# tunabrain/tungsten

Measured on AMD Instinct MI355X. Metric: Msamples/s (W*H*spp/s), path_tracer render loop, higher is better.
Workload: dtype f32; 1 GPU; materialtest.json (3 meshes 80768 tris + quad, smooth_coat/rough_conductor/lambert, envmap MIS) 1280x720 @ 256 spp; width=1280, height=720, spp=256, sampler=uniform (counter-based PCG), adaptive_sampling=False, max_bounces=64, parallelism=tile-shard x1

## Files before the change

tungsten_amd/csrc/hip/pt_wavefront.h:

```cpp
#ifndef TGAMD_PT_WAVEFRONT_H_
#define TGAMD_PT_WAVEFRONT_H_
#include "pt_kernels.h"

#include <hip/hip_runtime.h>

#include <cstdio>
#include <cstdlib>
#include <cstring>
#include <mutex>
#include <string>
#include <type_traits>
#include <vector>


#ifdef PT_PROFILE
#define PROF_DECL unsigned long long profT = wall_clock64(), profAcc[16] = {0, 0, 0, 0, 0, 0, 0, 0, 0, 0, 0, 0, 0, 0, 0, 0}, profLn[16] = {0, 0, 0, 0, 0, 0, 0, 0, 0, 0, 0, 0, 0, 0, 0, 0}
#define PROF(n) do { unsigned long long t_ = wall_clock64(); profAcc[n] += t_ - profT; profLn[n] += (t_ - profT)*(unsigned long long)__popcll(__ballot(true)); profT = t_; if ((n) == 0) profAcc[10]++; } while (0)
#define PROF_FLUSH(stats) do { if (laneId() == 0) for (int k_ = 0; k_ < 16; ++k_) if (k_ != 11) { if (k_ != 10) atomicAdd(&(stats).prof[k_], profAcc[k_]); atomicAdd(&(stats).profCls[cls][k_], profAcc[k_]); atomicAdd(&(stats).profLanes[cls][k_], profLn[k_]); } } while (0)
#else
#define PROF_DECL
#define PROF(n)
#define PROF_FLUSH(stats)
#endif

// ... 315 lines not shown
        }
        if (busyMask == 0ull)
            break;
        bool pop = false;
        if (busy && cur >= 0) {
            const float4 *nd = &at32(s.nodes, (uint32_t)cur*4u);
            float4 n0 = ld4(nd, 0u), n1 = ld4(nd, 1u), n2 = ld4(nd, 2u), n3 = ld4(nd, 3u);
            if (COUNT) nodes++;
            float e0, e1;
            bool h0 = boxTest(mk3(n0.x, n0.y, n0.z), mk3(n0.w, n1.x, n1.y), ray, invD, tmax, e0);
            bool h1 = boxTest(mk3(n1.z, n1.w, n2.x), mk3(n2.y, n2.z, n2.w), ray, invD, tmax, e1);
            int c0 = __float_as_int(n3.x), c1 = __float_as_int(n3.y);
            if (h0 && h1) {
                if (e1 < e0) { stack[sp*stride] = c0; cur = c1; }
                else { stack[sp*stride] = c1; cur = c0; }
                sp++;
            } else if (h0) { cur = c0; }
            else if (h1) { cur = c1; }
            else pop = true;
        }
        {
            unsigned long long atLeaf = __ballot(busy && cur < 0 && !pop);
            unsigned long long atNode = __ballot(busy && (cur >= 0 || pop));
            if (atLeaf != 0ull && ((uint32_t)__popcll(atLeaf) >= st.leaf_batch_bvh2 || atNode == 0ull)) {
                if (busy && cur < 0 && !pop) {
                    uint32_t firstRec = TGHIP_LEAF_FIRST(cur), count = TGHIP_LEAF_COUNT(cur);
                    for (uint32_t r = firstRec; r < firstRec + count; ++r) {
                        if (COUNT) prims++;
                        uint32_t meta;
                        (void)testRecord<false, SOLIDS ? KINDS_ALL : KINDS_MESH>(s, r, ray, tmax, hit, meta);
                    }
                    pop = true;
                }
            }
        }
        if (busy && pop) {
            if (sp == 0) {
                slotF4(st, A_HIT, slot) = hit;
                int ri = __float_as_int(hit.w);
                int cls = ri < 0 ? CLS_MISS : (int)at32(s.rec_class, (uint32_t)ri);
                queuePush(true, local, L, shadeQueue(cls));
                busy = false;
            } else {
                sp--;
                cur = stack[sp*stride];
            }
        }
    }
    waveAddStat(&L.closest_rays, rays);
    if (COUNT) { waveAddStat(&L.nodes, nodes); waveAddStat(&L.prims, prims); }
    queuesEnd(L, st, Q_EXT, Q_SHADE_MASK, Q_EXTP);
    if (threadIdx.x == 0) {
        ctl.closest_rays += L.closest_rays;
        if (COUNT) { st.stats[blockIdx.x].nodes_visited += L.nodes; st.stats[blockIdx.x].prims_tested += L.prims; }
    }
}

template<bool COUNT, bool SOLIDS = true>
__global__ __launch_bounds__(512) void k_trace_closest_inst(DeviceScene s, PathState st)
{
    extern __shared__ int ldsDyn[];
    __shared__ BlockLdsSmall L;
    __shared__ uint32_t fetchNext;
    unsigned short *order = reinterpret_cast<unsigned short *>(ldsDyn);
    int *stack = ldsDyn + (st.slots_per_block >> 1) + threadIdx.x;
    const int stride = (int)blockDim.x;
    BlockCtl &ctl = st.ctl[blockIdx.x];
    if (threadIdx.x == 0) fetchNext = 0;
    queuesBegin(L, st, ctl, Q_EXTP, 0u, order, Q_EXT);
    const uint32_t n = L.n;
    const uint32_t first = blockIdx.x*st.slots_per_block;
    uint32_t nodes = 0, prims = 0, rays = 0;
    constexpr uint32_t KINDS = SOLIDS ? KINDS_ALL : KINDS_MESH;

    bool busy = false;
    uint32_t slot = 0, local = 0;
    RayD world; world.o = splat3(0.0f); world.d = splat3(1.0f); world.tmin = 0.0f; world.tmax = 0.0f;
    RayD ray = world;
    f3 invD = splat3(1.0f), winvD = splat3(1.0f);
    float tmax = 0.0f;
    float4 hit = make_float4(0.0f, 0.0f, 0.0f, __int_as_float(-1));
    int hitInst = -1;
    int cur = 0, sp = 0, level = 0;
    float refTMin = 0.0f, refTMax = 0.0f, refFarT = 0.0f;
    int refSp = 0;
    uint32_t leafNext = 0, leafEnd = 0;
    int instSp = 0, curInst = -1;
    float ltmax = 0.0f;
    float4 lhit = hit;
    bool exhausted = false;
    uint32_t sec[24] = {0, 0, 0, 0, 0, 0, 0, 0, 0, 0, 0, 0, 0, 0, 0, 0, 0, 0, 0, 0, 0, 0, 0, 0};
#define INST_SECTION(k, pred) do { if (COUNT) { const unsigned long long m_ = __ballot(pred); if (m_) { sec[2*(k)]++; sec[2*(k) + 1] += (uint32_t)__popcll(m_); } } } while (0)
    for (;;) {
        unsigned long long busyMask = __ballot(busy);
        if (!exhausted && __popcll(busyMask) <= 48) {
            INST_SECTION(11, !busy);
            unsigned long long want = ~busyMask;
            uint32_t lane = laneId();
            uint32_t base = 0;
            if (lane == 0)
                base = atomicAdd(&fetchNext, (uint32_t)__popcll(want));
            base = __shfl(base, 0);
            if (!busy) {
                uint32_t i = base + __popcll(want & ((1ull << lane) - 1ull));
                if (i < n) {
                    local = order[i];
                    slot = first + local;
                    float4 ro = slotF4(st, A_RAY_O, slot), rd = slotF4(st, A_RAY_D, slot);
                    world.o = xyz(ro); world.d = xyz(rd); world.tmin = ro.w; world.tmax = rd.w;
                    ray = world;
                    winvD = mk3(1.0f/world.d.x, 1.0f/world.d.y, 1.0f/world.d.z);
                    invD = winvD;
                    tmax = world.tmax;
                    hit = make_float4(tmax, 0.0f, 0.0f, __int_as_float(-1));
                    hitInst = -1;
                    cur = 0; sp = 0; level = 0;
                    busy = true;
                    rays++;
                }
            }
            if (base + (uint32_t)__popcll(want) >= n)
                exhausted = true;
            busyMask = __ballot(busy);
        }
        if (busyMask == 0ull)
            break;
        bool pop = false;
        INST_SECTION(0, busy);
        INST_SECTION(1, busy && cur >= 0);
        INST_SECTION(2, busy && cur >= 0 && level == 1);
        if (busy && cur >= 0) {
            const float4 *nd = &at32(s.nodes, (uint32_t)cur*4u);
            const float4 n0 = ld4(nd, 0u), n1 = ld4(nd, 1u), n2 = ld4(nd, 2u), n3 = ld4(nd, 3u);
            if (COUNT) nodes++;
            const f3 lo0 = mk3(n0.x, n0.y, n0.z), hi0 = mk3(n0.w, n1.x, n1.y), lo1 = mk3(n1.z, n1.w, n2.x), hi1 = mk3(n2.y, n2.z, n2.w);
            const int c0 = __float_as_int(n3.x), c1 = __float_as_int(n3.y);
            float e0, e1;
            bool h0, h1, firstIs1;
            if (level == 1) {
                h0 = refChildTest(lo0, hi0, world.o, world.d, winvD, world.tmin, refFarT, e0);
                h1 = refChildTest(lo1, hi1, world.o, world.d, winvD, world.tmin, refFarT, e1);
                firstIs1 = !(e0 < e1);
            } else {
                const float far = level == 2 ? ltmax : tmax;
                h0 = boxTest(lo0, hi0, ray, invD, far, e0);
                h1 = boxTest(lo1, hi1, ray, invD, far, e1);
                firstIs1 = e1 < e0;
            }
            float entry = 0.0f;
            if (h0 && h1) {
                stack[sp*stride] = firstIs1 ? c0 : c1;
                sp++;
                cur = firstIs1 ? c1 : c0;
                entry = firstIs1 ? e1 : e0;
            } else if (h0) { cur = c0; entry = e0; }
            else if (h1) { cur = c1; entry = e1; }
            else pop = true;
            if (level == 1 && !pop) refTMin = entry;
        }
        {
            unsigned long long atLeaf = __ballot(busy && cur < 0 && !pop);
            unsigned long long atNode = __ballot(busy && (cur >= 0 || pop));
            if (atLeaf != 0ull && ((uint32_t)__popcll(atLeaf) >= st.leaf_batch_bvh2 || atNode == 0ull)) {
                INST_SECTION(3, busy && cur < 0 && !pop);
                INST_SECTION(4, busy && cur < 0 && !pop && level == 1);
                INST_SECTION(6, busy && cur < 0 && !pop && level != 1);
                if (busy && cur < 0 && !pop) {
                    if (level == 1) {
                        if (leafNext == leafEnd) { leafNext = TGHIP_LEAF_FIRST(cur); leafEnd = leafNext + TGHIP_LEAF_COUNT(cur); }
                        const uint32_t ri = s.inst_prims[leafNext];
                        leafNext++;
                        if (COUNT) prims++;
                        if (instanceReachable(s, ri, world, winvD, refTMin)) {
                            int root;
                            instanceLocalRay(s, ri, world, refTMin, PT_INF, ray, root);
                            invD = mk3(1.0f/ray.d.x, 1.0f/ray.d.y, 1.0f/ray.d.z);
                            ltmax = PT_INF;
                            lhit = make_float4(PT_INF, 0.0f, 0.0f, __int_as_float(-1));
                            curInst = (int)ri;
                            instSp = sp;
                            stack[sp*stride] = cur;
                            sp++;
                            cur = root;
                            level = 2;
                        } else if (leafNext == leafEnd) {
                            refTMax = refMin(refTMax, tmax);
                            refFarT = refTMax;
                            leafNext = leafEnd = 0;
                            pop = true;
                        }
                    } else {
                        const uint32_t firstRec = TGHIP_LEAF_FIRST(cur), count = TGHIP_LEAF_COUNT(cur);
                        bool entered = false;
                        if (level == 0) {
                            const float4 r0 = ld4(s.recs, firstRec*3u);
                            INST_SECTION(5, TGHIP_REC_KIND(__float_as_uint(r0.w)) == TGHIP_REC_INSTANCE_SET);
                            if (TGHIP_REC_KIND(__float_as_uint(r0.w)) == TGHIP_REC_INSTANCE_SET) {
                                if (COUNT) prims++;
                                const float4 r1 = ld4(s.recs, firstRec*3u + 1u), r2 = ld4(s.recs, firstRec*3u + 2u);
                                float tMin = world.tmin, tMax = tmax;
                                if (refBboxIntersection(xyz(r0), xyz(r1), world, tMin, tMax)) {
                                    refTMin = tMin; refTMax = tMax; refFarT = tmax;
                                    refSp = sp;
                                    leafNext = leafEnd = 0;
                                    cur = __float_as_int(r2.x);
                                    level = 1;
                                } else {
                                    pop = true;
                                }
                                entered = true;
                            }
                        }
                        if (!entered) {
                            for (uint32_t r = firstRec; r < firstRec + count; ++r) {
                                if (COUNT) prims++;
                                uint32_t meta;
                                if (level == 2) (void)testRecord<false, KINDS>(s, r, ray, ltmax, lhit, meta);
                                else if (testRecord<false, KINDS>(s, r, ray, tmax, hit, meta)) hitInst = -1;
                            }
                            pop = true;
                        }
                    }
                }
            }
        }
        INST_SECTION(7, busy && pop);
        INST_SECTION(8, busy && pop && level == 2 && sp == instSp + 1);
        if (busy && pop) {
            if (level == 2 && sp == instSp + 1) {
                if (__float_as_int(lhit.w) >= 0) { hit = lhit; hitInst = curInst; tmax = lhit.x; }
                ray = world; invD = winvD;
                level = 1;
                sp--;
                cur = stack[sp*stride];
                if (leafNext == leafEnd) {
                    refTMax = refMin(refTMax, tmax);
                    refFarT = refTMax;
                    leafNext = leafEnd = 0;
                } else {
                    pop = false;
                }
            }
            INST_SECTION(9, pop && level == 1);
            if (pop && level == 1) {
                for (;;) {
                    if (sp == refSp) { level = 0; break; }
                    sp--;
                    cur = stack[sp*stride];
                    if (cur >= 0) { pop = false; break; }
                    refTMin = refLeafEntry(s, TGHIP_LEAF_FIRST(cur), world.o, world.d, winvD, world.tmin);
                    if (!(refTMax < refTMin)) { pop = false; break; }
                }
            }
            INST_SECTION(10, pop && level != 1 && sp == 0);
            if (pop && level != 1) {
                if (sp == 0) {
                    slotF4(st, A_HIT, slot) = hit;
                    slotW(st, A_EMI, slot, 3u) = __int_as_float(hitInst);
                    int ri = __float_as_int(hit.w);
                    int cls = ri < 0 ? CLS_MISS : (int)at32(s.rec_class, (uint32_t)ri);
                    queuePush(true, local, L, shadeQueue(cls));
                    busy = false;
                } else {
                    sp--;
                    cur = stack[sp*stride];
                }
            }
        }
    }
    if (COUNT && laneId() == 0) {
        unsigned long long *wk = st.stats[blockIdx.x].walk[0];
        atomicAdd(&wk[4], 1ull);
        for (int k = 0; k < 24; ++k) atomicAdd(&wk[24 + k], (unsigned long long)sec[k]);
    }
#undef INST_SECTION
    waveAddStat(&L.closest_rays, rays);
    if (COUNT) { waveAddStat(&L.nodes, nodes); waveAddStat(&L.prims, prims); }
    queuesEnd(L, st, Q_EXT, Q_SHADE_MASK, Q_EXTP);
    if (threadIdx.x == 0) {
        ctl.closest_rays += L.closest_rays;
        if (COUNT) { st.stats[blockIdx.x].nodes_visited += L.nodes; st.stats[blockIdx.x].prims_tested += L.prims; }
    }
}

#ifndef PT_CLOSEST_WAVES
#define PT_CLOSEST_WAVES 5
#endif
#ifndef WIDE_CLOSEST_BOUNDS
#define WIDE_CLOSEST_BOUNDS __launch_bounds__(512, PT_CLOSEST_WAVES)
#endif
#ifndef WIDE_SHADOW_BOUNDS
#define WIDE_SHADOW_BOUNDS __launch_bounds__(512, 4)
#endif
#define PT_TURN_JOIN() asm volatile("" ::: "memory")
#define PT_WALK_FETCH(s, r0, r1, r2, nd, hasRec, recIdx, hasNode, nodeIdx) do { \
        const uint32_t recAt_ = (hasRec) ? (recIdx)*3u : 0u; \
        const uint32_t nodeAt_ = (hasNode) ? wideNodeOff(s, nodeIdx) : 0u; \
        r0 = at32((s).recs, recAt_); r1 = at32((s).recs, recAt_ + 1u); r2 = at32((s).recs, recAt_ + 2u); \
        wideNodeFetch(nd, reinterpret_cast<const char *>((s).wide), nodeAt_); \
    } while (0)
#ifndef PT_REFILL_AT
#define PT_REFILL_AT 40
#endif
template<bool COUNT, bool SOLIDS, bool INST, bool DECOUPLED, int NTS = PT_NT_STATE>
PT_DEV void traceClosestWideBody(const DeviceScene &s, const PathState &st, BlockLds &L, uint32_t &fetchNext, int *ldsDyn)
{
    unsigned short *order = reinterpret_cast<unsigned short *>(ldsDyn);
    uint2 *stack = reinterpret_cast<uint2 *>(ldsDyn + (st.slots_per_block >> 1)) + threadIdx.x;
    const int stride = (int)blockDim.x;
    BlockCtl &ctl = st.ctl[blockIdx.x];
    if (threadIdx.x == 0) fetchNext = 0;
    const unsigned long long wpStart = COUNT ? wall_clock64() : 0ull;
    queuesBegin(L, st, ctl, Q_EXTP, 0u, order, Q_EXT);
    const uint32_t n = L.n;
    const uint32_t first = blockIdx.x*st.slots_per_block;
    uint32_t nodes = 0, prims = 0, rays = 0;
    uint32_t turns = 0, dryTurns = 0;

    bool busy = false;
    uint32_t slot = 0, local = 0;
    RayD ray; ray.o = splat3(0.0f); ray.d = splat3(1.0f); ray.tmin = 0.0f; ray.tmax = 0.0f;
    WideRay wr; wr.idir = splat3(1.0f); wr.octInv = 0u;
    WideState w;
    wideStart(w);
    float tmax = 0.0f;
    float4 hit = make_float4(0.0f, 0.0f, 0.0f, __int_as_float(-1));
    int hitInst = -1;
    bool pendingPublish = false;
    bool exhausted = false;
    uint32_t age = 0;
    const bool maySuspend = !INST && st.suspend_lanes != 0u && n >= st.suspend_min_queue;
    WALK_PROF_DECL;
    for (;;) {
        unsigned long long busyMask = __ballot(busy);
        if constexpr (DECOUPLED) {
            const unsigned long long pendMask = __ballot(pendingPublish);
            if (pendMask != 0ull && ((!exhausted && __popcll(busyMask) <= PT_REFILL_AT) || (exhausted && (__popcll(pendMask) > 8 || busyMask == 0ull)))) {
                WALK_SECTION(wpPubs, wpPubLanes, pendingPublish);
                if (pendingPublish) {
                    slotF4<NTS>(st, A_HIT, slot) = hit;
                    const int ri = __float_as_int(hit.w);
                    const int cls = ri < 0 ? CLS_MISS : (int)at32(s.rec_class, (uint32_t)ri);
                    queuePush(true, local, L, shadeQueue(cls));
                    pendingPublish = false;
                }
            }
        }
        if (!exhausted && __popcll(busyMask) <= PT_REFILL_AT) {
            unsigned long long want = ~busyMask;
            uint32_t lane = laneId();
            uint32_t base = 0;
            if (lane == 0)
                base = atomicAdd(&fetchNext, (uint32_t)__popcll(want));
            base = __shfl(base, 0);
            WALK_SECTION(wpRefills, wpRefillLanes, !busy && base + __popcll(want & ((1ull << lane) - 1ull)) < n);
            if (!busy) {
                uint32_t i = base + __popcll(want & ((1ull << lane) - 1ull));
                if (i < n) {
                    local = order[i];
                    slot = first + local;
                    float4 ro = slotF4<NTS>(st, A_RAY_O, slot), rd = slotF4<NTS>(st, A_RAY_D, slot);
                    ray.o = xyz(ro); ray.d = xyz(rd); ray.tmin = ro.w; ray.tmax = rd.w;
                    bool resumed = false;
                    if constexpr (!INST) {
                        resumed = (__float_as_uint(ro.w) & WALK_SUSPENDED_BIT) != 0u;
                        ray.tmin = __uint_as_float(__float_as_uint(ro.w) & ~WALK_SUSPENDED_BIT);
                    }
                    wr = wideRaySetup(ray);
                    if (!resumed) {
                        wideStart(w);
                        tmax = ray.tmax;
                        hit = make_float4(tmax, 0.0f, 0.0f, __int_as_float(-1));
                        if constexpr (DECOUPLED && !INST) {
                            if (s.hoisted_rec >= 0) {
                                uint32_t meta;
                                if (COUNT) prims++;
                                (void)testRecord<true, KIND_BIT(TGHIP_REC_QUAD)>(s, (uint32_t)s.hoisted_rec, ray, tmax, hit, meta);
                            }
                        }
                        rays++;
                        if (COUNT) wpRays++;
                    } else {
                        walkRestore(st, slot, w, stack, stride);
                        if (COUNT) wpResumed++;
                        hit = slotF4<NTS>(st, A_HIT, slot);
                        tmax = hit.x;
                        slotW(st, A_RAY_O, slot, 3u) = ray.tmin;
                    }
                    hitInst = -1;
                    age = 0;
                    busy = true;
                }
            }
            if (base + (uint32_t)__popcll(want) >= n) {
                exhausted = true;
                if (COUNT) wpDry = wall_clock64();
            }
            busyMask = __ballot(busy);
        }
        if constexpr (!INST) {
            if (maySuspend && exhausted && (uint32_t)__popcll(busyMask) <= st.suspend_lanes) {
                if (busy && age >= st.suspend_turns) {
                    walkSave(st, slot, w, stack, stride);
                    if (COUNT) wpSuspended++;
                    slotF4<NTS>(st, A_HIT, slot) = hit;
                    slotW(st, A_RAY_O, slot, 3u) = __uint_as_float(__float_as_uint(ray.tmin) | WALK_SUSPENDED_BIT);
                    queuePush(true, local, L, Q_EXT);
                    busy = false;
                }
                busyMask = __ballot(busy);
            }
        }
        if (busyMask == 0ull) {
            if (DECOUPLED && __ballot(pendingPublish) != 0ull)
                continue;
            break;
        }
        age++;
        if (COUNT) { turns++; dryTurns += exhausted ? 1u : 0u; if (exhausted) wpBusyDry += (uint32_t)__popcll(busyMask); else wpBusy += (uint32_t)__popcll(busyMask); }
        if constexpr (!INST && DECOUPLED) {
            uint32_t recIdx = 0, nodeIdx = 0;
            bool hasRec = false, hasNode = false, finished = false;
            if (busy) {
                if (w.triMask == 0u && w.tri2Mask != 0u) { w.triBase = w.tri2Base; w.triMask = w.tri2Mask; w.triValid = w.tri2Valid; w.tri2Mask = 0u; }
                if (w.triMask) {
                    const uint32_t b = (uint32_t)__ffs((int)w.triMask) - 1u;
                    recIdx = w.triBase + (uint32_t)__popc(w.triValid & ((1u << b) - 1u));
                    w.triMask &= w.triMask - 1u;
                    hasRec = true;
                }
                if (w.tri2Mask == 0u)
                    hasNode = wideNextNode(w, wr.octInv, stack, stride, nodeIdx);
            }
            float4 r0, r1, r2;
            WideNodeRegs nd;
            PT_WALK_FETCH(s, r0, r1, r2, nd, hasRec, recIdx, hasNode, nodeIdx);
            WALK_SECTION(wpRecTurns, wpRecLanes, hasRec);
            WALK_SECTION(wpNodeTurns, wpNodeLanes, hasNode);
            if (hasRec) {
                if (COUNT) prims++;
                uint32_t meta;
                const bool accepted = testRecordLoaded<false, SOLIDS ? KINDS_ALL : KINDS_MESH>(s, recIdx, r0, r1, r2, ray, tmax, hit, meta);
                if (COUNT && accepted) wpHits++;
            }
            if (hasNode) {
                if (COUNT) nodes++;
                const uint32_t ob = w.triBase, om = w.triMask, ov = w.triValid;
                wideVisit(w, nd, ray.o, wr, ray.tmin, tmax, s.hoisted_rec >= 0);
                if (om) { w.tri2Base = w.triBase; w.tri2Mask = w.triMask; w.tri2Valid = w.triValid; w.triBase = ob; w.triMask = om; w.triValid = ov; }
            }
            if (busy && wideWalkOver(w)) {
                busy = false;
                pendingPublish = true;
            }
            (void)finished;
        } else if constexpr (!INST) {
            uint32_t recIdx = 0, nodeIdx = 0;
            bool hasRec = false, hasNode = false, finished = false;
            if (busy) {
                uint32_t idx = 0;
                const int what = wideNext<false>(w, wr.octInv, stack, stride, idx);
                if (what == 1) {
                    hasRec = true; recIdx = idx;
                    if (w.triMask == 0u && st.leaf_batch != 9u) {
                        const int next = wideNext<false>(w, wr.octInv, stack, stride, idx);
                        if (next == 2) { hasNode = true; nodeIdx = idx; } else finished = true;
                    }
                } else if (what == 2) { hasNode = true; nodeIdx = idx; }
                else finished = true;
            }
            float4 r0, r1, r2;
            WideNodeRegs nd;
            if (hasRec) { r0 = at32(s.recs, recIdx*3u + 0u); r1 = at32(s.recs, recIdx*3u + 1u); r2 = at32(s.recs, recIdx*3u + 2u); }
            if (hasNode) wideNodeFetch(nd, reinterpret_cast<const char *>(s.wide), wideNodeOff(s, nodeIdx));
            if (hasRec) {
                if (COUNT) prims++;
                uint32_t meta;
                (void)testRecordLoaded<false, SOLIDS ? KINDS_ALL : KINDS_MESH>(s, recIdx, r0, r1, r2, ray, tmax, hit, meta);
            }
            if (hasNode) {
                if (COUNT) nodes++;
                wideVisit(w, nd, ray.o, wr, ray.tmin, tmax);
            }
            if (finished) {
                slotF4<NTS>(st, A_HIT, slot) = hit;
                int ri = __float_as_int(hit.w);
                int cls = ri < 0 ? CLS_MISS : (int)at32(s.rec_class, (uint32_t)ri);
                queuePush(true, local, L, shadeQueue(cls));
                busy = false;
            }
        } else {
            uint32_t idx = 0;
            int what = 0;
            if (busy) {
                const bool wantsRecord = w.triMask != 0u;
                bool go = true;
                if (st.leaf_batch != 1u) {
                    const uint32_t nRec = (uint32_t)__popcll(__ballot(wantsRecord)), nNode = (uint32_t)__popcll(__ballot(!wantsRecord));
                    go = (nRec*st.leaf_batch >= nNode*2u) == wantsRecord;
                }
                if (go) {
                    what = wideNext<INST>(w, wr.octInv, stack, stride, idx);
                    if (what == 0) {
                        slotF4<NTS>(st, A_HIT, slot) = hit;
                        if (INST) slotW(st, A_EMI, slot, 3u) = __int_as_float(hitInst);
                        int ri = __float_as_int(hit.w);
                        int cls = ri < 0 ? CLS_MISS : (int)at32(s.rec_class, (uint32_t)ri);
                        queuePush(true, local, L, shadeQueue(cls));
                        busy = false;
                    }
                }
            }
            if (INST && what == 3) {
                float4 ro = slotF4<NTS>(st, A_RAY_O, slot), rd = slotF4<NTS>(st, A_RAY_D, slot);
                ray.o = xyz(ro); ray.d = xyz(rd);
                wr = wideRaySetup(ray);
                w.curInst = -1;
            } else if (what != 0) {
                const uint32_t off = what != 1 ? wideNodeOff(s, idx) : s.recs_offset + idx*48u;
                const float4 *p = reinterpret_cast<const float4 *>(reinterpret_cast<const char *>(s.wide) + (size_t)off);
                float4 q0 = p[0], q1 = p[1], q2 = p[2];
                if (what == 2) {
                    WideNodeRegs nd;
                    wideNodeFetchRest(nd, reinterpret_cast<const char *>(s.wide), off, q0, q1, q2);
                    if (COUNT) nodes++;
                    wideVisit(w, nd, ray.o, wr, ray.tmin, tmax);
                } else if (INST && what == 4) {
                    wideResumeRecords(w, idx, q1);
                } else {
                    if (COUNT) prims++;
                    if (INST && TGHIP_REC_KIND(__float_as_uint(q0.w)) == TGHIP_REC_INSTANCE) {
                        wideEnterInstance(w, stack, stride, idx, q0, q1, q2, ray, wr);
                    } else {
                        uint32_t meta;
                        if (testRecordLoaded<false, SOLIDS ? KINDS_ALL : KINDS_MESH>(s, idx, q0, q1, q2, ray, tmax, hit, meta))
                            hitInst = w.curInst;
                    }
                }
            }
            PT_TURN_JOIN();
            }
    }
    if (COUNT) wpLoopEnd = wall_clock64();
    waveAddStat(&L.closest_rays, rays);
    if (COUNT) { waveAddStat(&L.nodes, nodes); waveAddStat(&L.prims, prims); }
    queuesEnd(L, st, Q_EXT, Q_SHADE_MASK, Q_EXTP);
    if (threadIdx.x == 0) {
        ctl.closest_rays += L.closest_rays;
        if (COUNT) { st.stats[blockIdx.x].nodes_visited += L.nodes; st.stats[blockIdx.x].prims_tested += L.prims; }
    }
    if (COUNT && laneId() == 0) { atomicAdd(&st.stats[blockIdx.x].prof[10], (unsigned long long)turns); atomicAdd(&st.stats[blockIdx.x].prof[11], (unsigned long long)dryTurns); }
    if (COUNT) WALK_PROF_FLUSH(0, turns - dryTurns, dryTurns);
}
template<bool COUNT, bool SOLIDS = true, bool INST = false, bool DECOUPLED = false>
__global__ WIDE_CLOSEST_BOUNDS void k_trace_closest_wide(DeviceScene s, PathState st)
{
    extern __shared__ int ldsDyn[];
    __shared__ BlockLds L;
    __shared__ uint32_t fetchNext;
    traceClosestWideBody<COUNT, SOLIDS, INST, DECOUPLED>(s, st, L, fetchNext, ldsDyn);
}
template<int NTS = PT_NT_STATE>
PT_DEV bool finishBody(const DeviceScene &s, const PathState &st, const PassParams &pp, BlockLds &L, unsigned short *order);
template<bool COUNT, bool SOLIDS>
__global__ WIDE_CLOSEST_BOUNDS void k_finish_trace_closest_wide(DeviceScene s, PathState st, PassParams pp)
{
    extern __shared__ int ldsDyn[];
    __shared__ BlockLds L;
    __shared__ uint32_t fetchNext;
    (void)finishBody(s, st, pp, L, reinterpret_cast<unsigned short *>(ldsDyn));
    __syncthreads();
    traceClosestWideBody<COUNT, SOLIDS, false, true>(s, st, L, fetchNext, ldsDyn);
}

template<bool COUNT, bool SOLIDS = true>
__global__ __launch_bounds__(512) void k_trace_closest_instw(DeviceScene s, PathState st)
{
    extern __shared__ int ldsDyn[];
    __shared__ BlockLdsSmall L;
    __shared__ uint32_t fetchNext;
    unsigned short *order = reinterpret_cast<unsigned short *>(ldsDyn);
    int *stack = ldsDyn + (st.slots_per_block >> 1) + threadIdx.x;
    const int stride = (int)blockDim.x;
    uint2 *wstack = reinterpret_cast<uint2 *>(ldsDyn + (((st.slots_per_block >> 1) + st.inst_tree_depth*blockDim.x + 1u) & ~1u)) + threadIdx.x;
    BlockCtl &ctl = st.ctl[blockIdx.x];
    if (threadIdx.x == 0) fetchNext = 0;
    queuesBegin(L, st, ctl, Q_EXTP, 0u, order, Q_EXT);
    const uint32_t n = L.n;
    const uint32_t first = blockIdx.x*st.slots_per_block;
    uint32_t nodes = 0, wnodes = 0, prims = 0, rays = 0;
    constexpr uint32_t KINDS = SOLIDS ? KINDS_ALL : KINDS_MESH;
    const uint32_t phaseMin = st.inst_phase_min;

    bool busy = false;
    uint32_t slot = 0, local = 0;
    RayD world; world.o = splat3(0.0f); world.d = splat3(1.0f); world.tmin = 0.0f; world.tmax = 0.0f;
    f3 winvD = splat3(1.0f);
    RayD ray = world;
    WideRay wr; wr.idir = splat3(1.0f); wr.octInv = 0u;
    WideState w;
    wideStart(w);
    float tmax = 0.0f;
    float4 hit = make_float4(0.0f, 0.0f, 0.0f, __int_as_float(-1));
    int hitInst = -1;
    int cur = 0, sp = 0, level = 0;
    float refTMin = 0.0f, refTMax = 0.0f, refFarT = 0.0f;
    int refSp = 0;
    uint32_t leafNext = 0, leafEnd = 0;
    int curInst = -1;
    float ltmax = 0.0f;
    float4 lhit = hit;
    bool popPending = false;
    bool exhausted = false;
    uint32_t sec[24] = {0, 0, 0, 0, 0, 0, 0, 0, 0, 0, 0, 0, 0, 0, 0, 0, 0, 0, 0, 0, 0, 0, 0, 0};
#define INST_SECTION(k, pred) do { if (COUNT) { const unsigned long long m_ = __ballot(pred); if (m_) { sec[2*(k)]++; sec[2*(k) + 1] += (uint32_t)__popcll(m_); } } } while (0)
    for (;;) {
        unsigned long long busyMask = __ballot(busy);
        if (!exhausted && (uint32_t)__popcll(busyMask) <= st.inst_refill_at) {
            INST_SECTION(11, !busy);
            unsigned long long want = ~busyMask;
            uint32_t lane = laneId();
            uint32_t base = 0;
            if (lane == 0)
                base = atomicAdd(&fetchNext, (uint32_t)__popcll(want));
            base = __shfl(base, 0);
            if (!busy) {
                uint32_t i = base + __popcll(want & ((1ull << lane) - 1ull));
                if (i < n) {
                    local = order[i];
                    slot = first + local;
                    float4 ro = slotF4(st, A_RAY_O, slot), rd = slotF4(st, A_RAY_D, slot);
                    world.o = xyz(ro); world.d = xyz(rd); world.tmin = ro.w; world.tmax = rd.w;
                    winvD = mk3(1.0f/world.d.x, 1.0f/world.d.y, 1.0f/world.d.z);
                    tmax = world.tmax;
                    hit = make_float4(tmax, 0.0f, 0.0f, __int_as_float(-1));
                    hitInst = -1;
                    cur = 0; sp = 0; level = 0;
                    popPending = false;
                    busy = true;
                    rays++;
                }
            }
            if (base + (uint32_t)__popcll(want) >= n)
                exhausted = true;
            busyMask = __ballot(busy);
        }
        if (busyMask == 0ull)
            break;
        const bool inMaster = busy && level == 2;
        const uint32_t nM = (uint32_t)__popcll(__ballot(inMaster)), nT = (uint32_t)__popcll(busyMask) - nM;
        const bool runM = nM != 0u && (nM >= nT || nM >= phaseMin);
        const bool runT = nT != 0u && (nT > nM || nT >= phaseMin);
        INST_SECTION(0, busy);
        if (runM) {
            INST_SECTION(1, inMaster);
            uint32_t recIdx = 0, nodeIdx = 0;
            bool hasRec = false, hasNode = false;
            if (inMaster) {
                if (w.triMask == 0u && w.tri2Mask != 0u) { w.triBase = w.tri2Base; w.triMask = w.tri2Mask; w.triValid = w.tri2Valid; w.tri2Mask = 0u; }
                if (w.triMask) {
                    const uint32_t b = (uint32_t)__ffs((int)w.triMask) - 1u;
                    recIdx = w.triBase + (uint32_t)__popc(w.triValid & ((1u << b) - 1u));
                    w.triMask &= w.triMask - 1u;
                    hasRec = true;
                }
                if (w.tri2Mask == 0u)
                    hasNode = wideNextNode(w, wr.octInv, wstack, stride, nodeIdx);
            }
            float4 r0, r1, r2;
            WideNodeRegs nd;
            PT_WALK_FETCH(s, r0, r1, r2, nd, hasRec, recIdx, hasNode, nodeIdx);
            INST_SECTION(2, hasRec);
            INST_SECTION(3, hasNode);
            if (hasRec) {
                if (COUNT) prims++;
                uint32_t meta;
                (void)testRecordLoaded<false, KINDS>(s, recIdx, r0, r1, r2, ray, ltmax, lhit, meta);
            }
            if (hasNode) {
                if (COUNT) wnodes++;
                const uint32_t ob = w.triBase, om = w.triMask, ov = w.triValid;
                wideVisit(w, nd, ray.o, wr, ray.tmin, ltmax);
                if (om) { w.tri2Base = w.triBase; w.tri2Mask = w.triMask; w.tri2Valid = w.triValid; w.triBase = ob; w.triMask = om; w.triValid = ov; }
            }
            const bool masterDone = inMaster && wideWalkOver(w);
            INST_SECTION(4, masterDone);
            if (masterDone) {
                if (__float_as_int(lhit.w) >= 0) { hit = lhit; hitInst = curInst; tmax = lhit.x; }
                level = 1;
                if (leafNext == leafEnd) {
                    refTMax = refMin(refTMax, tmax);
                    refFarT = refTMax;
                    leafNext = leafEnd = 0;
                    popPending = true;
                }
            }
        }
        if (runT) {
            const bool inTree = busy && level != 2;
            INST_SECTION(5, inTree);
            bool pop = inTree && popPending;
            popPending = inTree ? false : popPending;
            INST_SECTION(6, inTree && !pop && cur >= 0);
            if (inTree && !pop && cur >= 0) {
                const float4 *nd = &at32(s.nodes, (uint32_t)cur*4u);
                const float4 n0 = ld4(nd, 0u), n1 = ld4(nd, 1u), n2 = ld4(nd, 2u), n3 = ld4(nd, 3u);
                if (COUNT) nodes++;
                const f3 lo0 = mk3(n0.x, n0.y, n0.z), hi0 = mk3(n0.w, n1.x, n1.y), lo1 = mk3(n1.z, n1.w, n2.x), hi1 = mk3(n2.y, n2.z, n2.w);
                const int c0 = __float_as_int(n3.x), c1 = __float_as_int(n3.y);
                float e0, e1;
                bool h0, h1, firstIs1;
                if (level == 1) {
                    h0 = refChildTest(lo0, hi0, world.o, world.d, winvD, world.tmin, refFarT, e0);
                    h1 = refChildTest(lo1, hi1, world.o, world.d, winvD, world.tmin, refFarT, e1);
                    firstIs1 = !(e0 < e1);
                } else {
                    h0 = boxTest(lo0, hi0, world, winvD, tmax, e0);
                    h1 = boxTest(lo1, hi1, world, winvD, tmax, e1);
                    firstIs1 = e1 < e0;
                }
                float entry = 0.0f;
                if (h0 && h1) {
                    stack[sp*stride] = firstIs1 ? c0 : c1;
                    sp++;
                    cur = firstIs1 ? c1 : c0;
                    entry = firstIs1 ? e1 : e0;
                } else if (h0) { cur = c0; entry = e0; }
                else if (h1) { cur = c1; entry = e1; }
                else pop = true;
                if (level == 1 && !pop) refTMin = entry;
            }
            {
                const unsigned long long atLeaf = __ballot(inTree && cur < 0 && !pop);
                const unsigned long long atNode = __ballot(inTree && (cur >= 0 || pop));
                if (atLeaf != 0ull && ((uint32_t)__popcll(atLeaf) >= st.leaf_batch_bvh2 || atNode == 0ull)) {
                    INST_SECTION(7, inTree && cur < 0 && !pop);
                    INST_SECTION(8, inTree && cur < 0 && !pop && level == 1);
                    if (inTree && cur < 0 && !pop) {
                        if (level == 1) {
                            if (leafNext == leafEnd) { leafNext = TGHIP_LEAF_FIRST(cur); leafEnd = leafNext + TGHIP_LEAF_COUNT(cur); }
                            const uint32_t ri = s.inst_prims[leafNext];
                            leafNext++;
                            if (COUNT) prims++;
                            const bool reach = instanceReachable(s, ri, world, winvD, refTMin);
                            INST_SECTION(9, reach);
                            if (reach) {
                                const float4 q0 = ld4(s.recs, ri*3u + 0u), q1 = ld4(s.recs, ri*3u + 1u), q2 = ld4(s.recs, ri*3u + 2u);
                                const f3 qc = -xyz(q1);
                                ray.o = quatRotate(q1.w, qc, world.o - xyz(q0));
                                ray.d = quatRotate(q1.w, qc, world.d);
                                ray.tmin = refTMin; ray.tmax = PT_INF;
                                wr = wideRaySetup(ray);
                                wideStart(w);
                                w.node = (int)__float_as_uint(q2.z);
                                ltmax = PT_INF;
                                lhit = make_float4(PT_INF, 0.0f, 0.0f, __int_as_float(-1));
                                curInst = (int)ri;
                                level = 2;
                            } else if (leafNext == leafEnd) {
// ... 1814 lines not shown
```

Before: 1212 Msamples/s.

## Split decoupled closest-hit walk loop and overlap refill setup with fetches

Gives the decoupled non-instanced closest-hit traversal its own loop. A freshly refilled ray now issues its root-node fetch in the same turn, and the ray setup and hoisted-quad test run after the fetches are issued, so load latency overlaps with setup work. The hoisted quad record and its normal are loaded once per kernel into registers instead of being refetched per ray. The shade-queue push for finished rays is also deferred until after the fetch issue. The cost is more code and register pressure in a kernel bounded at 5 waves, plus subtle suspend/resume state handling, for example the w.node=-1 root trick and the resumed-path hasNode reset.

```diff
diff --git a/tungsten_amd/csrc/hip/pt_wavefront.h b/tungsten_amd/csrc/hip/pt_wavefront.h
--- a/tungsten_amd/csrc/hip/pt_wavefront.h
+++ b/tungsten_amd/csrc/hip/pt_wavefront.h
@@ -641,6 +641,35 @@
 #ifndef PT_REFILL_AT
 #define PT_REFILL_AT 40
 #endif
+struct HoistedQuad { float4 r0, r1, r2; f3 n; };
+PT_DEV HoistedQuad hoistedQuadLoad(const DeviceScene &s)
+{
+    HoistedQuad q;
+    q.r0 = q.r1 = q.r2 = make_float4(0.0f, 0.0f, 0.0f, 0.0f);
+    q.n = splat3(0.0f);
+    if (s.hoisted_rec >= 0) {
+        const PT_CONST_AS float *rp = asConst(reinterpret_cast<const float *>(s.recs)) + (uint32_t)s.hoisted_rec*12;
+        q.r0 = make_float4(rp[0], rp[1], rp[2], rp[3]);
+        q.r1 = make_float4(rp[4], rp[5], rp[6], rp[7]);
+        q.r2 = make_float4(rp[8], rp[9], rp[10], rp[11]);
+        const uint32_t meta = __float_as_uint(q.r0.w);
+        if (TGHIP_REC_KIND(meta) == TGHIP_REC_QUAD)
+            q.n = ld3(asConst(s.objects)[TGHIP_REC_OBJECT(meta)].normal);
+    }
+    return q;
+}
+PT_DEV bool hoistedQuadTest(const HoistedQuad &q, uint32_t ri, const RayD &ray, float &tmax, float4 &hit, uint32_t &hitMeta)
+{
+    const uint32_t meta = __float_as_uint(q.r0.w);
+    float t, u = 0.0f, v = 0.0f;
+    const bool ok = TGHIP_REC_KIND(meta) == TGHIP_REC_QUAD && quadTest(xyz(q.r0), xyz(q.r1), xyz(q.r2), q.r1.w, q.r2.w, q.n, ray, tmax, t, u, v);
+    if (ok) {
+        tmax = t;
+        hit = make_float4(t, u, v, __int_as_float((int)ri));
+        hitMeta = meta;
+    }
+    return ok;
+}
 template<bool COUNT, bool SOLIDS, bool INST, bool DECOUPLED, int NTS = PT_NT_STATE>
 PT_DEV void traceClosestWideBody(const DeviceScene &s, const PathState &st, BlockLds &L, uint32_t &fetchNext, int *ldsDyn)
 {
@@ -665,26 +694,141 @@
     float tmax = 0.0f;
     float4 hit = make_float4(0.0f, 0.0f, 0.0f, __int_as_float(-1));
     int hitInst = -1;
-    bool pendingPublish = false;
     bool exhausted = false;
     uint32_t age = 0;
     const bool maySuspend = !INST && st.suspend_lanes != 0u && n >= st.suspend_min_queue;
     WALK_PROF_DECL;
-    for (;;) {
-        unsigned long long busyMask = __ballot(busy);
-        if constexpr (DECOUPLED) {
+    if constexpr (!INST && DECOUPLED) {
+        const HoistedQuad hq = hoistedQuadLoad(s);
+        bool pendingPublish = false;
+        for (;;) {
+            unsigned long long busyMask = __ballot(busy);
+            const bool refill = !exhausted && __popcll(busyMask) <= PT_REFILL_AT;
             const unsigned long long pendMask = __ballot(pendingPublish);
-            if (pendMask != 0ull && ((!exhausted && __popcll(busyMask) <= PT_REFILL_AT) || (exhausted && (__popcll(pendMask) > 8 || busyMask == 0ull)))) {
+            bool pushing = false;
+            uint32_t pushLocal = 0u;
+            uint8_t pushCls = (uint8_t)CLS_MISS;
+            if (pendMask != 0ull && (refill || (exhausted && (__popcll(pendMask) > 8 || busyMask == 0ull)))) {
                 WALK_SECTION(wpPubs, wpPubLanes, pendingPublish);
                 if (pendingPublish) {
                     slotF4<NTS>(st, A_HIT, slot) = hit;
                     const int ri = __float_as_int(hit.w);
-                    const int cls = ri < 0 ? CLS_MISS : (int)at32(s.rec_class, (uint32_t)ri);
-                    queuePush(true, local, L, shadeQueue(cls));
+                    if (ri >= 0) pushCls = at32(s.rec_class, (uint32_t)ri);
+                    pushLocal = local;
+                    pushing = true;
                     pendingPublish = false;
                 }
             }
-        }
+            auto finishPublish = [&]() { if (pushing) queuePush(true, pushLocal, L, shadeQueue((int)pushCls)); };
+            bool fresh = false;
+            if (refill) {
+                unsigned long long want = ~busyMask;
+                uint32_t lane = laneId();
+                uint32_t base = 0;
+                if (lane == 0)
+                    base = atomicAdd(&fetchNext, (uint32_t)__popcll(want));
+                base = __shfl(base, 0);
+                const uint32_t i = base + __popcll(want & ((1ull << lane) - 1ull));
+                WALK_SECTION(wpRefills, wpRefillLanes, !busy && i < n);
+                if (!busy && i < n) {
+                    local = order[i];
+                    slot = first + local;
+                    const float4 ro = slotF4<NTS>(st, A_RAY_O, slot), rd = slotF4<NTS>(st, A_RAY_D, slot);
+                    ray.o = xyz(ro); ray.d = xyz(rd); ray.tmin = ro.w; ray.tmax = rd.w;
+                    age = 0;
+                    busy = true;
+                    fresh = true;
+                }
+                if (base + (uint32_t)__popcll(want) >= n) {
+                    exhausted = true;
+                    if (COUNT) wpDry = wall_clock64();
+                }
+                busyMask = __ballot(busy);
+            }
+            if (maySuspend && exhausted && (uint32_t)__popcll(busyMask) <= st.suspend_lanes) {
+                if (busy && age >= st.suspend_turns) {
+                    walkSave(st, slot, w, stack, stride);
+                    if (COUNT) wpSuspended++;
+                    slotF4<NTS>(st, A_HIT, slot) = hit;
+                    slotW(st, A_RAY_O, slot, 3u) = __uint_as_float(__float_as_uint(ray.tmin) | WALK_SUSPENDED_BIT);
+                    queuePush(true, local, L, Q_EXT);
+                    busy = false;
+                }
+                busyMask = __ballot(busy);
+            }
+            if (busyMask == 0ull) {
+                finishPublish();
+                if (__ballot(pendingPublish) != 0ull)
+                    continue;
+                break;
+            }
+            age++;
+            if (COUNT) { turns++; dryTurns += exhausted ? 1u : 0u; if (exhausted) wpBusyDry += (uint32_t)__popcll(busyMask); else wpBusy += (uint32_t)__popcll(busyMask); }
+            uint32_t recIdx = 0, nodeIdx = 0;
+            bool hasRec = false, hasNode = fresh;
+            if (busy && !fresh) {
+                if (w.triMask == 0u && w.tri2Mask != 0u) { w.triBase = w.tri2Base; w.triMask = w.tri2Mask; w.triValid = w.tri2Valid; w.tri2Mask = 0u; }
+                if (w.triMask) {
+                    const uint32_t b = (uint32_t)__ffs((int)w.triMask) - 1u;
+                    recIdx = w.triBase + (uint32_t)__popc(w.triValid & ((1u << b) - 1u));
+                    w.triMask &= w.triMask - 1u;
+                    hasRec = true;
+                }
+                if (w.tri2Mask == 0u)
+                    hasNode = wideNextNode(w, wr.octInv, stack, stride, nodeIdx);
+            }
+            float4 r0, r1, r2;
+            WideNodeRegs nd;
+            PT_WALK_FETCH(s, r0, r1, r2, nd, hasRec, recIdx, hasNode, nodeIdx);
+            finishPublish();
+            if (fresh) {
+                const bool resumed = (__float_as_uint(ray.tmin) & WALK_SUSPENDED_BIT) != 0u;
+                ray.tmin = __uint_as_float(__float_as_uint(ray.tmin) & ~WALK_SUSPENDED_BIT);
+                wr = wideRaySetup(ray);
+                if (!resumed) {
+                    wideStart(w);
+                    w.node = -1;
+                    tmax = ray.tmax;
+                    hit = make_float4(tmax, 0.0f, 0.0f, __int_as_float(-1));
+                    if (s.hoisted_rec >= 0) {
+                        uint32_t meta;
+                        if (COUNT) prims++;
+                        (void)hoistedQuadTest(hq, (uint32_t)s.hoisted_rec, ray, tmax, hit, meta);
+                    }
+                    rays++;
+                    if (COUNT) wpRays++;
+                } else {
+                    hasNode = false;
+                    age = 0;
+                    walkRestore(st, slot, w, stack, stride);
+                    if (COUNT) wpResumed++;
+                    hit = slotF4<NTS>(st, A_HIT, slot);
+                    tmax = hit.x;
+                    slotW(st, A_RAY_O, slot, 3u) = ray.tmin;
+                }
+            }
+            WALK_SECTION(wpRecTurns, wpRecLanes, hasRec);
+            WALK_SECTION(wpNodeTurns, wpNodeLanes, hasNode);
+            if (hasRec) {
+                if (COUNT) prims++;
+                uint32_t meta;
+                const bool accepted = testRecordLoaded<false, SOLIDS ? KINDS_ALL : KINDS_MESH>(s, recIdx, r0, r1, r2, ray, tmax, hit, meta);
+                if (COUNT && accepted) wpHits++;
+            }
+            if (hasNode) {
+                if (COUNT) nodes++;
+                const uint32_t ob = w.triBase, om = w.triMask, ov = w.triValid;
+                wideVisit(w, nd, ray.o, wr, ray.tmin, tmax, s.hoisted_rec >= 0);
+                if (om) { w.tri2Base = w.triBase; w.tri2Mask = w.triMask; w.tri2Valid = w.triValid; w.triBase = ob; w.triMask = om; w.triValid = ov; }
+            }
+            if (busy && wideWalkOver(w)) {
+                busy = false;
+                pendingPublish = true;
+            }
+        }
+    } else
+    for (;;) {
+        unsigned long long busyMask = __ballot(busy);
         if (!exhausted && __popcll(busyMask) <= PT_REFILL_AT) {
             unsigned long long want = ~busyMask;
             uint32_t lane = laneId();
@@ -710,13 +854,6 @@
                         wideStart(w);
                         tmax = ray.tmax;
                         hit = make_float4(tmax, 0.0f, 0.0f, __int_as_float(-1));
-                        if constexpr (DECOUPLED && !INST) {
-                            if (s.hoisted_rec >= 0) {
-                                uint32_t meta;
-                                if (COUNT) prims++;
-                                (void)testRecord<true, KIND_BIT(TGHIP_REC_QUAD)>(s, (uint32_t)s.hoisted_rec, ray, tmax, hit, meta);
-                            }
-                        }
                         rays++;
                         if (COUNT) wpRays++;
                     } else {
@@ -750,50 +887,11 @@
                 busyMask = __ballot(busy);
             }
         }
-        if (busyMask == 0ull) {
-            if (DECOUPLED && __ballot(pendingPublish) != 0ull)
-                continue;
+        if (busyMask == 0ull)
             break;
-        }
         age++;
         if (COUNT) { turns++; dryTurns += exhausted ? 1u : 0u; if (exhausted) wpBusyDry += (uint32_t)__popcll(busyMask); else wpBusy += (uint32_t)__popcll(busyMask); }
-        if constexpr (!INST && DECOUPLED) {
-            uint32_t recIdx = 0, nodeIdx = 0;
-            bool hasRec = false, hasNode = false, finished = false;
-            if (busy) {
-                if (w.triMask == 0u && w.tri2Mask != 0u) { w.triBase = w.tri2Base; w.triMask = w.tri2Mask; w.triValid = w.tri2Valid; w.tri2Mask = 0u; }
-                if (w.triMask) {
-                    const uint32_t b = (uint32_t)__ffs((int)w.triMask) - 1u;
-                    recIdx = w.triBase + (uint32_t)__popc(w.triValid & ((1u << b) - 1u));
-                    w.triMask &= w.triMask - 1u;
-                    hasRec = true;
-                }
-                if (w.tri2Mask == 0u)
-                    hasNode = wideNextNode(w, wr.octInv, stack, stride, nodeIdx);
-            }
-            float4 r0, r1, r2;
-            WideNodeRegs nd;
-            PT_WALK_FETCH(s, r0, r1, r2, nd, hasRec, recIdx, hasNode, nodeIdx);
-            WALK_SECTION(wpRecTurns, wpRecLanes, hasRec);
-            WALK_SECTION(wpNodeTurns, wpNodeLanes, hasNode);
-            if (hasRec) {
-                if (COUNT) prims++;
-                uint32_t meta;
-                const bool accepted = testRecordLoaded<false, SOLIDS ? KINDS_ALL : KINDS_MESH>(s, recIdx, r0, r1, r2, ray, tmax, hit, meta);
-                if (COUNT && accepted) wpHits++;
-            }
-            if (hasNode) {
-                if (COUNT) nodes++;
-                const uint32_t ob = w.triBase, om = w.triMask, ov = w.triValid;
-                wideVisit(w, nd, ray.o, wr, ray.tmin, tmax, s.hoisted_rec >= 0);
-                if (om) { w.tri2Base = w.triBase; w.tri2Mask = w.triMask; w.tri2Valid = w.triValid; w.triBase = ob; w.triMask = om; w.triValid = ov; }
-            }
-            if (busy && wideWalkOver(w)) {
-                busy = false;
-                pendingPublish = true;
-            }
-            (void)finished;
-        } else if constexpr (!INST) {
+        if constexpr (!INST) {
             uint32_t recIdx = 0, nodeIdx = 0;
             bool hasRec = false, hasNode = false, finished = false;
             if (busy) {
```

New measurement: 1230 Msamples/s (median of 6 runs). +1.5%, better.
